# LouisBearing/BirdSoundClassif

Hardware: AMD Instinct MI355X
Metric: clips/sec (3 s @ 22.05 kHz) detect fwd (higher is better)
Workload: dtype f32; 1 GPU; BASELINE.json configs[1]: 1xMI355X inference, batch=64 synthetic 3 s clips (PCM16 @22.05 kHz resident in HBM) through the HIP STFT front end + detector forward + device post-processing, detections returned to the host; batch_per_gpu=64, distinct_clips=64, lanes=2

## Files before the change

### birdsoundclassif_amd/_lib.py

```python
import ctypes as C
import os
import subprocess

_HERE = os.path.dirname(os.path.abspath(__file__))
LIB_PATH = os.environ.get('NBM_LIB') or os.path.join(_HERE, 'libnbm_hip.so')
CSRC = os.path.join(_HERE, 'csrc')

_lib = None


class GemmDesc(C.Structure):
    _fields_ = [('x', C.c_void_p), ('w', C.c_void_p), ('y', C.c_void_p),
                ('scale', C.c_void_p), ('shift', C.c_void_p), ('residual', C.c_void_p),
                ('x_gs', C.c_int64), ('w_gs', C.c_int64), ('y_gs', C.c_int64), ('res_gs', C.c_int64),
                ('groups', C.c_int),
                ('B', C.c_int), ('H', C.c_int), ('W', C.c_int), ('Cin', C.c_int),
                ('N', C.c_int),
                ('kh', C.c_int), ('kw', C.c_int), ('stride', C.c_int), ('pad', C.c_int),
                ('Ho', C.c_int), ('Wo', C.c_int),
                ('x_ld', C.c_int), ('w_ld', C.c_int), ('y_ld', C.c_int), ('res_ld', C.c_int),
                ('alpha', C.c_float), ('act', C.c_int), ('shift_per_row', C.c_int),
                ('up', C.c_void_p), ('up_H', C.c_int), ('up_W', C.c_int),
                ('rows', C.c_void_p), ('rows_blocks', C.c_void_p),
                ('rows_mode', C.c_int), ('rows_count', C.c_int), ('rows_TH', C.c_int), ('rows_TW', C.c_int),
# ... 114 lines not shown
    'nbm_leaky_relu_bwd': [_P, _P, _P, _F, _L, _P],
    'nbm_layernorm_bwd': [_P, _P, _P, _L, _I, _F, _P, _P, _P, _P],
    'nbm_mha_small_bwd': [_P, _P, _P, _P, _I, _I, _I, _I, _P, _P, _P, _I, _I, _I, _P, _I, _I, _I, _I, _L, _L, _P, _F, _P],
    'nbm_layernorm_bwd_det': [_P, _P, _P, _L, _I, _F, _P, _P, _P, _P, _L, _P],
    'nbm_dropout': [_P, _P, _P, _L, _U32, _F, _U64, _U32, _U32, _P],
    'nbm_mha_small_drop': [_P, _P, _P, _I, _I, _I, _P, _I, _I, _I, _I, _I, _L, _L, _P, _F, _U32, _F, _U64, _U32, _U32, _P],
    'nbm_mha_small_drop_bwd': [_P, _P, _P, _P, _I, _I, _I, _I, _P, _P, _P, _I, _I, _I, _P, _I, _I, _I, _I, _L, _L, _P, _F,
                               _U32, _F, _U64, _U32, _U32, _P],
    'nbm_zero_roi_windows': [_P, _I, _I, _I, _P, _P, _I, _I, _I, _P],
    'nbm_zero_pattern': [_P, _I, _I, _I, _I, _I, _P],
    'nbm_zero_tiles': [_P, _I, _I, _I, _I, _P, _I, _P, _P],
    'nbm_tiles_gather': [_P, _I, _I, _I, _I, _P, _I, _P, _P, _P],
    'nbm_tiles_scatter_add': [_P, _I, _I, _I, _I, _P, _I, _P, _P, _P],
    'nbm_proposal_iou': [_P, _P, _P, _I, _I, _I, _P, _P, _P],
    'nbm_anchor_targets': [_P, _I, _P, _P, _I, _I, _F, _F, _P, _P, _P, _P],
    'nbm_maxpool3x3s2_bwd': [_P, _P, _P, _I, _I, _I, _I, _I, _I, _P, _P, _P],
    'nbm_upsample_bilinear_bwd': [_P, _I, _I, _I, _I, _P, _I, _I, _I, _P],
    'nbm_tiles_upsample_bilinear_bwd_add': [_P, _I, _I, _I, _I, _P, _I, _P, _P, _I, _I, _P],
    'nbm_png_unfilter_gray8': [_P, _L, _I, _I, _I, _P, _L, _P, _P],
    'nbm_png_inflate': [_P, _L, _P, _I, _P, _L, _L, _P, _P],
    'nbm_image_half_std_u8': [_P, _L, _I, _L, _P, _P],
    'nbm_randn_fill': [_U64, _L, _P, _P],
    'nbm_augment_batch': [_P, _P, _P, _I, _I, _I, _P, _P, _P, _P, _P, _P, _P],
    'nbm_u8_to_unit': [_P, _L, _P, _P],
    'nbm_wino_input': [_P, _I, _I, _I, _I, _P, _I, _P],
    'nbm_wino_output': [_P, _P, _P, _P, _I, _I, _I, _I, _I, _P, _I, _P, _P],
    'nbm_wino_outgrad': [_P, _I, _I, _I, _I, _P, _P, _I, _P],
    'nbm_wino_weight': [_P, _P, _I, _I, _I, _I, _P, _P],
    'nbm_wino_weight_grad': [_P, _P, _I, _I, _I, _P, _P],
    'nbm_wino23_rows': [_P, _I, _I, _I, _I, _P, _P],
    'nbm_wino23_conv_fused': [_P, _P, _P, _P, _P, _I, _I, _I, _I, _I, _I, _P, _I, _P],
    'nbm_wino23_rows_tiles': [_P, _I, _I, _I, _I, _P, _I, _P, _P, _P, _I, _P],
    'nbm_wino23_conv_fused_tiles': [_P, _P, _P, _P, _P, _I, _I, _I, _I, _I, _I, _P, _P, _I, _P, _P, _P],
    'nbm_roi_tiles': [_P, _P, _I, _I, _I, _I, _P, _P, _P, _I, _P, _P, _P],
    'nbm_wino23_input_tiles': [_P, _I, _I, _I, _I, _P, _I, _P, _P, _P],
    'nbm_wino23_outgrad_tiles': [_P, _I, _I, _I, _I, _P, _I, _P, _P, _P, _I, _P],
    'nbm_cell_outgrad': [_P, _I, _I, _I, _I, _I, _P, _P, _P],
    'nbm_cell_weight': [_P, _I, _I, _P, _I, _P, _I, _P],
    'nbm_cell_weight_fold': [_P, _P, _I, _I, _I, _I, _F, _P, _I, _P, _I, _P],
    'nbm_cell_weight_grad': [_P, _I, _I, _I, _P, _P],
    'nbm_cell_input': [_P, _I, _I, _I, _I, _I, _P, _I, _I, _P],
    'nbm_cell_input_up': [_P, _P, _I, _I, _I, _I, _I, _I, _I, _P, _I, _I, _P],
    'nbm_cell_patches': [_P, _I, _I, _I, _I, _I, _P, _I, _I, _P],
    'nbm_cell_patches_up': [_P, _P, _I, _I, _I, _I, _I, _I, _I, _P, _I, _I, _P],
    'nbm_cell_patches_up_cols': [_P, _P, _I, _I, _I, _I, _I, _I, _I, _P, _P],
    'nbm_cell_dgrad_output': [_P, _I, _I, _I, _I, _I, _P, _I, _I, _I, _P, _P],
    'nbm_cell_output': [_P, _P, _I, _I, _I, _I, _I, _P, _P],
    'nbm_weighted_sum': [_P, _P, _P, _P, _P, _L, _P],
    'nbm_weighted_sum_bwd': [_P, _P, _P, _P, _P, _P, _P, _P, _P, _L, _P],
    'nbm_softmax_rows_bwd': [_P, _P, _P, _L, _I, _F, _P],
    'nbm_pair_softmax_bwd': [_P, _P, _P, _L, _P],
    'nbm_dwconv3x3_bwd': [_P, _P, _P, _I, _I, _I, _I, _I, _I, _P, _P, _P, _I, _I, _P],
    'nbm_dwconv3x3_bwd_acc': [_P, _P, _I, _I, _I, _I, _I, _I, _P, _I, _I, _P],
    'nbm_film_fwd': [_P, _P, _P, _L, _I, _P],
    'nbm_film_bwd': [_P, _P, _P, _P, _P, _L, _I, _P],
    'nbm_bn_train_fwd': [_P, _L, _I, _P, _P, _F, _F, _P, _P, _P, _P, _P, _P, _P],
    'nbm_bn_train_bwd': [_P, _P, _L, _I, _P, _P, _P, _P, _P, _P, _P, _P],
    'nbm_bn_act_plan': [_L, _I, C.POINTER(C.c_int), C.POINTER(C.c_int64)],
    'nbm_bn_act_train_fwd': [_P, _L, _I, _P, _P, _F, _F, _P, _P, _P, _I, _P, _L, _P, _P, _P, _P],
    'nbm_bn_act_train_bwd': [_P, _P, _P, _L, _I, _P, _P, _P, _I, _P, _L, _P, _P, _P, _P, _P],
    'nbm_roi_pool_bwd': [C.POINTER(C.c_void_p), C.POINTER(C.c_int), C.POINTER(C.c_int), _I, _I, _P, _P, _I, _I, _P, _P],
    'nbm_roi_pool_hw_bwd': [C.POINTER(C.c_void_p), C.POINTER(C.c_int), C.POINTER(C.c_int), _I, _I, _P, _P, _I, _I, _I, _I, _P, _P],
    'nbm_sqnorm_accum': [_P, _L, _P, _P],
    'nbm_adamw_step': [_P, _P, _P, _P, _L, _F, _F, _F, _F, _F, _I, _P, _F, _P],
}

# ... 41 lines not shown
```

### birdsoundclassif_amd/csrc/wino_fused.hip

```cpp
#include "nbm_common.h"
#include "igemm_device.h"
#include <type_traits>

namespace {

constexpr int BK = 32;
constexpr int PITCH = 36;
constexpr int LIST_BM = 128;

struct WinoFusedParams {
  const float* R; const float* U; float* y;
  const float* scale; const float* shift; const float* mask;
  long long r_gs;
  int u_gs;
  int T, N, C, nk;
  int H, W, TH, TW, THW, WP;
  nbm_fastdiv fd_thw, fd_tw;
  int m_tiles, n_tiles, relu;
  const int* tiles; const int* n_blocks;
  const unsigned* blk_info;
};

__global__ __launch_bounds__(256) void wino23_rows_kernel(const float* __restrict__ x, int B, int H, int W, int C4,
                                                          int TH, int WP, float* __restrict__ R) {
  const long long per_plane = (long long)B * TH * WP * C4;
  const f32x4* x4 = reinterpret_cast<const f32x4*>(x);
  f32x4* r4 = reinterpret_cast<f32x4*>(R);
  const f32x4 zero = {0.f, 0.f, 0.f, 0.f};
  for (long long idx = blockIdx.x * 256ll + threadIdx.x; idx < per_plane; idx += (long long)gridDim.x * 256) {
    const int c = (int)(idx % C4);
    long long t = idx / C4;
    const int xp = (int)(t % WP);
    t /= WP;
    const int ty = (int)(t % TH), b = (int)(t / TH);
    const int ix = xp - 1;
    f32x4 d[4];
#pragma unroll
    for (int a = 0; a < 4; ++a) {
      const int iy = 2 * ty - 1 + a;
      const bool ok = (unsigned)iy < (unsigned)H && (unsigned)ix < (unsigned)W;
      d[a] = ok ? x4[(((long long)b * H + iy) * W + ix) * C4 + c] : zero;
    }
    r4[idx] = d[0] - d[2];
    r4[idx + per_plane] = d[1] + d[2];
    r4[idx + 2 * per_plane] = d[2] - d[1];
    r4[idx + 3 * per_plane] = d[1] - d[3];
  }
}

__global__ __launch_bounds__(256) void wino23_rows_tiles_kernel(const float* __restrict__ x, int B, int H, int W, int C4,
                                                                int TH, int TW, int WP, const int* __restrict__ tiles,
                                                                int n_entries, const int* __restrict__ n_blocks,
                                                                const unsigned* __restrict__ blk_info, float* __restrict__ R,
// ... 11 lines not shown
    const int k = (int)(t & 3), e = (int)(t >> 2);
    const int id = tiles[e];
    if (id < 0) continue;
    const unsigned pm = blk_info ? blk_info[e >> 7] & 0xffffu : 0xffffu;
    if ((k == 0 && !(pm & 0x1111u)) || (k == 3 && !(pm & 0x8888u))) continue;
    const int THW = TH * TW;
    const int b = id / THW, rem = id - b * THW;
    const int ty = rem / TW, tx = rem - ty * TW;
    const int xp = 2 * tx + k, ix = xp - 1;
    f32x4 d[4];
#pragma unroll
    for (int a = 0; a < 4; ++a) {
      const int iy = 2 * ty - 1 + a;
      bool ok = (unsigned)iy < (unsigned)H && (unsigned)ix < (unsigned)W &&
                !(a == 0 && !(pm & 0x000fu)) && !(a == 3 && !(pm & 0xf000u));
      if (S > 0 && ok && (iy + 1) % S < 3 && (iy + 1) / S < OHp && (ix + 1) % S < 3 && (ix + 1) / S < OWp) ok = false;
      d[a] = ok ? x4[(((long long)b * H + iy) * W + ix) * C4 + c] : zero;
    }
    const long long o = (((long long)b * TH + ty) * WP + xp) * C4 + c;
    if (pm & 0x000fu) r4[o] = d[0] - d[2];
    r4[o + per_plane] = d[1] + d[2];
    r4[o + 2 * per_plane] = d[2] - d[1];
    if (pm & 0xf000u) r4[o + 3 * per_plane] = d[1] - d[3];
  }
}

template <int BM, int BN, int WM, int WN>
__global__ __launch_bounds__(256, BN == 128 ? 1 : 2) void wino23_fused_kernel(const WinoFusedParams p) {
  constexpr int MT = WM / 32, NT = WN / 32;
  constexpr int WAVES_N = BN / WN;
  constexpr int AR = BM / 32, BR = BN / 32;
  static_assert((BM / WM) * WAVES_N == 4, "4 waves per workgroup");

  __shared__ __attribute__((aligned(16))) float lds[2 * (BM + BN) * PITCH];
  if constexpr (BN != 128) nbm_stagger_priority();
  float* As = lds;
  float* Bs = lds + 2 * BM * PITCH;

  const int wg = xcd_tile(gridDim.x, blockIdx.x);
  int tile_m = wg / p.n_tiles, tile_n = wg - tile_m * p.n_tiles;
  if (p.n_blocks) {
    const int j = blockIdx.x >> 3;
    tile_n = j % p.n_tiles;
    tile_m = (j / p.n_tiles) * 8 + (blockIdx.x & 7);
    if (tile_m >= p.m_tiles) return;
  }
  const int bm0 = tile_m * BM, bn0 = tile_n * BN;

  if (p.tiles) {
    if (p.n_blocks && tile_m >= *p.n_blocks) return;
    if (p.tiles[bm0] < 0) return;
  }
  auto tile_of = [&](int t) { return p.tiles ? p.tiles[t] : t; };
  const unsigned info = (p.tiles && p.blk_info) ? p.blk_info[tile_m] : 0x000fffffu;
  const unsigned plane_mask = info & 0xffffu, store_mask = (info >> 16) & 0xfu;

  const int tid = threadIdx.x, lane = tid & 63, wave = tid >> 6;
  const int wm0 = (wave / WAVES_N) * WM, wn0 = (wave % WAVES_N) * WN;
  const int lrow = lane & 31, lh = lane >> 5;
  const int c4 = tid & 7, r0 = tid >> 3;

  unsigned a_rel[AR], b_rel[BR];
  long long blk_base;
  {
    const int t = bm0 < p.T ? tile_of(bm0) : 0;
    const int bi = (int)nbm_fdiv((unsigned)t, p.fd_thw), rem = t - bi * p.THW;
    const int ty = (int)nbm_fdiv((unsigned)rem, p.fd_tw), tx = rem - ty * p.TW;
    blk_base = (((long long)bi * p.TH + ty) * p.WP + 2 * tx) * p.C;
  }
#pragma unroll
  for (int i = 0; i < AR; ++i) {
    const int t = bm0 + r0 + 32 * i < p.T ? tile_of(bm0 + r0 + 32 * i) : -1;
    if (t >= 0) {
      const int bi = (int)nbm_fdiv((unsigned)t, p.fd_thw), rem = t - bi * p.THW;
      const int ty = (int)nbm_fdiv((unsigned)rem, p.fd_tw), tx = rem - ty * p.TW;
      const long long off = (((long long)bi * p.TH + ty) * p.WP + 2 * tx) * p.C - blk_base;
      a_rel[i] = (unsigned)((off + c4 * 4) * 4);
    } else {
      a_rel[i] = 0x80000000u;
    }
  }
#pragma unroll
  for (int i = 0; i < BR; ++i) {
    const int n = bn0 + r0 + 32 * i;
    b_rel[i] = n < p.N ? (unsigned)((n * p.C + c4 * 4) * 4) : 0x80000000u;
  }
  const float* a_plane0 = p.R + blk_base;
  const __amdgpu_buffer_rsrc_t rsrc_b = make_rsrc(p.U, 0x7ffffff0u);

  f32x4 ra[AR], ra2[AR], rb[BR];
  float a_sign = 1.f;
  unsigned ld_rem = plane_mask;
  int ld_xi = __builtin_ctz(ld_rem), ld_c0 = 0;

  auto load_tiles = [&]() {
    const int i = ld_xi >> 2, j = ld_xi & 3;
    const int k1 = j == 0 ? 0 : (j == 2 ? 2 : 1), k2 = j == 2 ? 1 : (j == 3 ? 3 : 2);
    const __amdgpu_buffer_rsrc_t rsrc_a = make_rsrc(a_plane0 + (long long)i * p.r_gs, 0x7ffffff0u);
    const unsigned a_soff1 = (unsigned)((k1 * p.C + ld_c0) * 4), a_soff2 = (unsigned)((k2 * p.C + ld_c0) * 4);
    const unsigned b_soff = (unsigned)((ld_xi * p.u_gs + ld_c0) * 4);
#pragma unroll
    for (int r = 0; r < AR; ++r) {
      ra[r] = __builtin_bit_cast(f32x4, __builtin_amdgcn_raw_buffer_load_b128(rsrc_a, a_rel[r], a_soff1, 0));
      ra2[r] = __builtin_bit_cast(f32x4, __builtin_amdgcn_raw_buffer_load_b128(rsrc_a, a_rel[r], a_soff2, 0));
    }
#pragma unroll
    for (int r = 0; r < BR; ++r)
      rb[r] = __builtin_bit_cast(f32x4, __builtin_amdgcn_raw_buffer_load_b128(rsrc_b, b_rel[r], b_soff, 0));
    ld_c0 += BK;
    if (ld_c0 == p.C) { ld_c0 = 0; ld_rem &= ld_rem - 1; ld_xi = ld_rem ? __builtin_ctz(ld_rem) : 0; }
  };
  unsigned st_rem = plane_mask;
  int st_xi = __builtin_ctz(st_rem), st_c0 = 0;
  auto store_lds = [&](int buf) {
    const float sgn = (st_xi & 3) == 1 ? 1.f : -1.f;
#pragma unroll
    for (int r = 0; r < AR; ++r) {
      f32x4 v;
#pragma unroll
      for (int e = 0; e < 4; ++e) v[e] = fmaf(sgn, ra2[r][e], ra[r][e]);
      *reinterpret_cast<f32x4*>(As + (buf * BM + r0 + 32 * r) * PITCH + c4 * 4) = v;
    }
#pragma unroll
    for (int r = 0; r < BR; ++r)
      *reinterpret_cast<f32x4*>(Bs + (buf * BN + r0 + 32 * r) * PITCH + c4 * 4) = rb[r];
    st_c0 += BK;
    if (st_c0 == p.C) { st_c0 = 0; st_rem &= st_rem - 1; st_xi = st_rem ? __builtin_ctz(st_rem) : 0; }
  };
  (void)a_sign;

  f32x16 acc[MT][NT];
  f32x16 Y[2][2][MT][NT];
#pragma unroll
  for (int i = 0; i < MT; ++i)
#pragma unroll
    for (int j = 0; j < NT; ++j)
#pragma unroll
      for (int e = 0; e < 16; ++e) {
        acc[i][j][e] = 0.f;
        Y[0][0][i][j][e] = 0.f; Y[0][1][i][j][e] = 0.f; Y[1][0][i][j][e] = 0.f; Y[1][1][i][j][e] = 0.f;
      }

  f32x4 fa[2][MT], fb[2][NT];
  auto read_frags = [&](const float* Ab, const float* Bb, int q, int s) {
#pragma unroll
    for (int i = 0; i < MT; ++i) fa[s][i] = *reinterpret_cast<const f32x4*>(Ab + i * 32 * PITCH + q * 4);
#pragma unroll
    for (int j = 0; j < NT; ++j) fb[s][j] = *reinterpret_cast<const f32x4*>(Bb + j * 32 * PITCH + q * 4);
  };
  auto mfma_group = [&](int s) {
#pragma unroll
    for (int e = 0; e < 4; ++e)
#pragma unroll
      for (int i = 0; i < MT; ++i)
#pragma unroll
        for (int j = 0; j < NT; ++j)
          acc[i][j] = __builtin_amdgcn_mfma_f32_32x32x2f32(fa[s][i][e], fb[s][j][e], acc[i][j], 0, 0, 0);
  };

  int cur = 0;
  auto k_step = [&](auto store_c, auto load_c) {
    constexpr bool STORE = decltype(store_c)::value, LOAD = decltype(load_c)::value;
    constexpr int NM = 4 * MT * NT;
    __syncthreads();
    const float* Ab = As + (cur * BM + wm0 + lrow) * PITCH + lh * 16;
    const float* Bb = Bs + (cur * BN + wn0 + lrow) * PITCH + lh * 16;
    read_frags(Ab, Bb, 0, 0);
    read_frags(Ab, Bb, 1, 1);
    mfma_group(0);
    if constexpr (STORE) store_lds(cur ^ 1);
    __builtin_amdgcn_sched_group_barrier(0x100, 2 * (MT + NT), 0);
    if constexpr (STORE) {
#pragma unroll
      for (int z = 0; z < AR + BR; ++z) {
        __builtin_amdgcn_sched_group_barrier(0x008, NM / (AR + BR) > 0 ? NM / (AR + BR) : 1, 0);
        __builtin_amdgcn_sched_group_barrier(0x200, 1, 0);
      }
    }
    __builtin_amdgcn_sched_barrier(0);
    read_frags(Ab, Bb, 2, 0);
    mfma_group(1);
    if constexpr (LOAD) load_tiles();
    __builtin_amdgcn_sched_group_barrier(0x100, MT + NT, 0);
    if constexpr (LOAD) {
#pragma unroll
      for (int z = 0; z < 2 * AR + BR; ++z) {
        __builtin_amdgcn_sched_group_barrier(0x008, 1, 0);
        __builtin_amdgcn_sched_group_barrier(0x002, 2, 0);
        __builtin_amdgcn_sched_group_barrier(0x020, 1, 0);
      }
    }
    __builtin_amdgcn_sched_barrier(0);
// ... 4 lines not shown
    __builtin_amdgcn_sched_barrier(0);
    mfma_group(1);
    cur ^= 1;
  };

  auto flush = [&](int xi) {
    const int i = xi >> 2, j = xi & 3;
    const float ai[2] = {i < 3 ? 1.f : 0.f, i == 0 ? 0.f : (i == 1 ? 1.f : -1.f)};
    const float aj[2] = {j < 3 ? 1.f : 0.f, j == 0 ? 0.f : (j == 1 ? 1.f : -1.f)};
#pragma unroll
    for (int pp = 0; pp < 2; ++pp)
#pragma unroll
      for (int qq = 0; qq < 2; ++qq) {
        const float c = ai[pp] * aj[qq];
        if (c != 0.f) {
#pragma unroll
          for (int a = 0; a < MT; ++a)
#pragma unroll
            for (int b = 0; b < NT; ++b)
#pragma unroll
              for (int e = 0; e < 16; ++e) Y[pp][qq][a][b][e] = fmaf(c, acc[a][b][e], Y[pp][qq][a][b][e]);
        }
      }
#pragma unroll
    for (int a = 0; a < MT; ++a)
#pragma unroll
      for (int b = 0; b < NT; ++b)
#pragma unroll
        for (int e = 0; e < 16; ++e) acc[a][b][e] = 0.f;
  };

  using TT = std::true_type;
  using FF = std::false_type;
  load_tiles();
  store_lds(0);
  load_tiles();
  for (unsigned rem = plane_mask; rem;) {
    const int xi = __builtin_ctz(rem);
    rem &= rem - 1;
    if (rem) {
      for (int kt = 0; kt < p.nk; ++kt) k_step(TT{}, TT{});
    } else {
      for (int kt = 0; kt + 2 < p.nk; ++kt) k_step(TT{}, TT{});
      k_step(TT{}, FF{});
      k_step(FF{}, FF{});
    }
    flush(xi);
  }
  __syncthreads();

  constexpr int CP = BN + 4;
  static_assert(BM * CP + 2 * BM <= 2 * (BM + BN) * PITCH, "epilogue tile + row table must fit the operand buffers");
  float* Cs = lds;
  long long* row_pix = reinterpret_cast<long long*>(lds + BM * CP);
  if (tid < BM) {
    const int t = bm0 + tid < p.T ? tile_of(bm0 + tid) : -1;
    long long v = -1;
    if (t >= 0) {
      const int bi = (int)nbm_fdiv((unsigned)t, p.fd_thw), rem = t - bi * p.THW;
      const int ty = (int)nbm_fdiv((unsigned)rem, p.fd_tw), tx = rem - ty * p.TW;
      const long long pix = (p.relu & 4) ? (long long)(bm0 + tid) * 4 : ((long long)bi * p.H + 2 * ty) * p.W + 2 * tx;
      v = (pix << 2) | (2 * ty + 1 < p.H ? 2 : 0) | (2 * tx + 1 < p.W ? 1 : 0);
    }
    row_pix[tid] = v;
  }
  constexpr int CH = BN / 4;
  constexpr int RPP = 256 / CH;
  const int cc = tid % CH, rr = tid / CH;
  const int n = bn0 + cc * 4;
  f32x4 sc = {1.f, 1.f, 1.f, 1.f}, sh = {0.f, 0.f, 0.f, 0.f};
  if (n < p.N) {
    if (p.scale) sc = *reinterpret_cast<const f32x4*>(p.scale + n);
    if (p.shift) sh = *reinterpret_cast<const f32x4*>(p.shift + n);
  }
#pragma unroll
  for (int pp = 0; pp < 2; ++pp)
#pragma unroll
    for (int qq = 0; qq < 2; ++qq) {
      if (!((store_mask >> (2 * pp + qq)) & 1u)) continue;
      __syncthreads();
#pragma unroll
      for (int a = 0; a < MT; ++a)
#pragma unroll
        for (int b = 0; b < NT; ++b)
#pragma unroll
          for (int e = 0; e < 16; ++e)
            Cs[(wm0 + a * 32 + (e & 3) + 8 * (e >> 2) + 4 * lh) * CP + wn0 + b * 32 + lrow] = Y[pp][qq][a][b][e];
      __syncthreads();
      if (n < p.N) {
        const int need = (pp ? 2 : 0) | (qq ? 1 : 0);
#pragma unroll 4
        for (int r = rr; r < BM; r += RPP) {
          const long long rp = row_pix[r];
          if (rp < 0) break;
          if ((rp & need) != need) continue;
          f32x4 v = *reinterpret_cast<const f32x4*>(Cs + r * CP + cc * 4);
          const long long idx = ((rp >> 2) + ((p.relu & 4) ? pp * 2 + qq : pp * p.W + qq)) * p.N + n;
#pragma unroll
          for (int e = 0; e < 4; ++e) v[e] = v[e] * sc[e] + sh[e];
          if (p.relu & 1) {
#pragma unroll
            for (int e = 0; e < 4; ++e) v[e] = fmaxf(v[e], 0.f);
          }
          if (p.relu & 2) {
            const f32x4 o = *reinterpret_cast<const f32x4*>(p.y + idx);
            v[0] += o[0]; v[1] += o[1]; v[2] += o[2]; v[3] += o[3];
          }
          if (p.mask) {
            const f32x4 mk = *reinterpret_cast<const f32x4*>(p.mask + idx);
#pragma unroll
            for (int e = 0; e < 4; ++e) if (!(mk[e] > 0.f)) v[e] = 0.f;
          }
          *reinterpret_cast<f32x4*>(p.y + idx) = v;
        }
      }
    }
}

}

extern "C" int nbm_wino23_rows(const float* x, int B, int H, int W, int C, float* R, void* stream) {
  if (!x || !R || B <= 0 || H <= 0 || W <= 0 || C <= 0 || (C & 3)) return NBM_EINVAL;
  if (!nbm_aligned16(x) || !nbm_aligned16(R)) return NBM_EALIGN;
  const int TH = (H + 1) >> 1, TW = (W + 1) >> 1, WP = 2 * TW + 2;
  const long long n = (long long)B * TH * WP * (C / 4);
  long long g = (n + 255) / 256;
  if (g > 65536) g = 65536;
  hipLaunchKernelGGL(wino23_rows_kernel, dim3((unsigned)g), dim3(256), 0, (hipStream_t)stream, x, B, H, W, C / 4, TH, WP, R);
  return nbm_launch_status();
}

extern "C" int nbm_wino23_rows_tiles(const float* x, int B, int H, int W, int C, const int* tiles, int n_entries,
                                     const int* n_blocks, const unsigned* blk_info, float* R, int skip_pattern_stride,
                                     void* stream) {
  if (!x || !R || !tiles || B <= 0 || H <= 0 || W <= 0 || C <= 0 || (C & 3) || n_entries < 0 || skip_pattern_stride < 0) return NBM_EINVAL;
  if (!nbm_aligned16(x) || !nbm_aligned16(R)) return NBM_EALIGN;
  if (n_entries == 0) return NBM_OK;
  const int TH = (H + 1) >> 1, TW = (W + 1) >> 1, WP = 2 * TW + 2;
  const long long n = (long long)n_entries * 4 * (C / 4);
  long long g = (n + 255) / 256;
  if (g > 16384) g = 16384;
  hipLaunchKernelGGL(wino23_rows_tiles_kernel, dim3((unsigned)g), dim3(256), 0, (hipStream_t)stream, x, B, H, W, C / 4, TH, TW,
                     WP, tiles, n_entries, n_blocks, blk_info, R, skip_pattern_stride);
  return nbm_launch_status();
}

static int wino23_conv_fused_launch(const float* R, const float* U, const float* scale, const float* shift,
                                    const float* mask, int relu, int B, int H, int W, int C, int N, float* y,
                                    const int* tiles, int n_entries, const int* n_blocks, const unsigned* blk_info,
                                    int variant, void* stream);

extern "C" int nbm_wino23_conv_fused(const float* R, const float* U, const float* scale, const float* shift,
                                     const float* mask, int relu, int B, int H, int W, int C, int N, float* y,
                                     int variant, void* stream) {
  return wino23_conv_fused_launch(R, U, scale, shift, mask, relu, B, H, W, C, N, y, nullptr, 0, nullptr, nullptr, variant, stream);
}

extern "C" int nbm_wino23_conv_fused_tiles(const float* R, const float* U, const float* scale, const float* shift,
                                           const float* mask, int relu, int B, int H, int W, int C, int N, float* y,
                                           const int* tiles, int n_entries, const int* n_blocks, const unsigned* blk_info,
                                           void* stream) {
  if (!tiles || n_entries < 0 || (n_entries % LIST_BM)) return NBM_EINVAL;
  if (n_entries == 0) return NBM_OK;
  return wino23_conv_fused_launch(R, U, scale, shift, mask, relu, B, H, W, C, N, y, tiles, n_entries, n_blocks, blk_info, 0,
                                  stream);
}

static int wino23_conv_fused_launch(const float* R, const float* U, const float* scale, const float* shift,
                                    const float* mask, int relu, int B, int H, int W, int C, int N, float* y,
                                    const int* tiles, int n_entries, const int* n_blocks, const unsigned* blk_info,
                                    int variant, void* stream) {
  if (!R || !U || !y || B <= 0 || H <= 0 || W <= 0 || C <= 0 || N <= 0) return NBM_EINVAL;
  if ((C % BK) || C / BK < 2 || (N & 3)) return NBM_EUNSUPPORTED;
  if (!nbm_aligned16(R) || !nbm_aligned16(U) || !nbm_aligned16(y) || (shift && !nbm_aligned16(shift)) ||
      (scale && !nbm_aligned16(scale)) || (mask && !nbm_aligned16(mask)))
    return NBM_EALIGN;
  WinoFusedParams p{};
  p.TH = (H + 1) >> 1; p.TW = (W + 1) >> 1; p.THW = p.TH * p.TW; p.WP = 2 * p.TW + 2;
  p.fd_thw = nbm_fastdiv_make((unsigned)p.THW); p.fd_tw = nbm_fastdiv_make((unsigned)p.TW);
  const long long T = (long long)B * p.THW;
  if (T > 0x7fffff00ll || (long long)N * C * 16 * 4 > 0x7fffffffll) return NBM_EUNSUPPORTED;
  if ((130ll * p.WP + 4) * C * 4 > 0x7fffffffll) return NBM_EUNSUPPORTED;
  if (tiles && (long long)(B < 8 ? B : 8) * p.TH * p.WP * C * 4 > 0x7fffffffll) return NBM_EUNSUPPORTED;
  p.R = R; p.U = U; p.y = y; p.scale = scale; p.shift = shift; p.mask = mask; p.relu = relu;
  p.T = (int)T; p.N = N; p.C = C; p.nk = C / BK; p.H = H; p.W = W;
  p.r_gs = (long long)B * p.TH * p.WP * C; p.u_gs = N * C;
  p.m_tiles = (int)((T + LIST_BM - 1) / LIST_BM);
  p.tiles = tiles; p.n_blocks = n_blocks; p.blk_info = blk_info;
  if (tiles) { p.T = n_entries; p.m_tiles = n_entries / LIST_BM; }
  hipStream_t st = (hipStream_t)stream;
  if (variant != 0 && variant != 64 && variant != 128) return NBM_EINVAL;
  const bool wide = variant == 128 || (variant == 0 && N % 128 == 0);
  p.n_tiles = wide ? (N + 127) / 128 : (N + 63) / 64;
  int bm = LIST_BM;
  if (wide && !tiles) {
    const char* fe = getenv("NBM_WINO_BM");
    const int force = fe ? atoi(fe) : 0;
    static const int cus = [] { int dev = 0, n = 0; (void)hipGetDevice(&dev); (void)hipDeviceGetAttribute(&n, hipDeviceAttributeMultiprocessorCount, dev);
                                return n > 0 ? n : 256; }();
    const long long nt = p.n_tiles;
    const long long r128 = ((T + 127) / 128 * nt + cus - 1) / cus, r96 = ((T + 95) / 96 * nt + cus - 1) / cus;
    if (force == 96 || (force == 0 && r96 * 96 * 108 < r128 * 128 * 100)) bm = 96;
    if (force == 128) bm = 128;
    p.m_tiles = (int)((T + bm - 1) / bm);
  }
  const dim3 grid((n_blocks ? (p.m_tiles + 7) / 8 * 8 : p.m_tiles) * p.n_tiles), block(256);
#define NBM_WF(BM_, BN_, WM_, WN_) hipLaunchKernelGGL((wino23_fused_kernel<BM_, BN_, WM_, WN_>), grid, block, 0, st, p)
  if (!wide) NBM_WF(128, 64, 64, 32);
  else if (bm == 96) NBM_WF(96, 128, 96, 32);
  else NBM_WF(128, 128, 64, 64);
#undef NBM_WF
  return nbm_launch_status();
}
```

### include/nbm_hip.h

```cpp
#ifndef NBM_HIP_H
#define NBM_HIP_H

#include <stdint.h>

#ifdef __cplusplus
extern "C" {
#endif

#define NBM_OK 0
#define NBM_EINVAL (-1)
#define NBM_EALIGN (-2)
#define NBM_EUNSUPPORTED (-3)

#define NBM_ACT_NONE 0
#define NBM_ACT_RELU 1
#define NBM_ACT_SILU 2
#define NBM_ACT_LEAKY 3

const char* nbm_version(void);

int nbm_graph_census(void* graph, long long counts[6]);

typedef struct nbm_gemm_desc {
  const float* x;
// ... 50 lines not shown
  long long workspace_bytes;
  int B, H, W;
  int groups, Cg;
  int kh, kw, stride, pad;
  int Ho, Wo;
  int g_ld, y_ld, x_ld, out_ld;
  int accumulate;
  int splits;
} nbm_gconv_bwd_desc;
int nbm_gconv3x3_dgrad(const nbm_gconv_bwd_desc* d, void* stream);
int nbm_gconv3x3_wgrad(const nbm_gconv_bwd_desc* d, void* stream);
int nbm_gconv3x3_wgrad_workspace(const nbm_gconv_bwd_desc* d, long long* bytes);

int nbm_wino_input(const float* x, int B, int H, int W, int C, float* V, int m, void* stream);
int nbm_wino_output(const float* M, const float* scale, const float* shift, const float* mask, int relu, int B, int H, int W,
                    int N, float* y, int m, const float* residual, void* stream);
int nbm_wino_outgrad(const float* g, int B, int H, int W, int N, float* dM, float* bias_grad, int m, void* stream);

int nbm_wino_weight(const float* g, const float* scale, int N, int C, int transposed, int m, float* U, void* stream);
int nbm_wino_weight_grad(const float* dU, const float* row_scale, int N, int C, int m, float* dW, void* stream);

int nbm_wino23_rows(const float* x, int B, int H, int W, int C, float* R, void* stream);
int nbm_wino23_conv_fused(const float* R, const float* U, const float* scale, const float* shift, const float* mask,
                          int relu, int B, int H, int W, int C, int N, float* y, int variant, void* stream);

int nbm_wino23_rows_tiles(const float* x, int B, int H, int W, int C, const int* tiles, int n_entries, const int* n_blocks,
                          const unsigned* blk_info, float* R,
                          int skip_pattern_stride ,
                          void* stream);
int nbm_wino23_conv_fused_tiles(const float* R, const float* U, const float* scale, const float* shift, const float* mask,
                                int relu ,
                                int B, int H, int W, int C, int N, float* y, const int* tiles, int n_entries,
                                const int* n_blocks, const unsigned* blk_info, void* stream);
int nbm_roi_tiles(const float* rois, const int* n_roi, int B, int roi_cap, int n_levels, int level, const int* fh,
                  const int* fw, const unsigned char* skip, int dilate, int* tiles, int* n_blocks, void* stream);
int nbm_wino23_input_tiles(const float* x, int B, int H, int W, int C, const int* tiles, int n_list, const unsigned* plane_mask,
                           float* V, void* stream);
int nbm_wino23_outgrad_tiles(const float* g, int B, int H, int W, int N, const int* tiles, int n_list, const unsigned* plane_mask,
                             float* dM, float* bias_grad, int skip_pattern_stride, void* stream);
int nbm_cell_outgrad(const float* g, int B, int H, int W, int N, int stride, float* Vg, float* bias_grad, void* stream);
int nbm_cell_weight(const float* w, int N, int C, float* U_nc, int ld, float* U_cn, int ldt, void* stream);
int nbm_cell_weight_fold(const float* w, const float* w_lat, int wl_ld, int N, int C, int Cin, float alpha, float* U_nc, int ld,
                         float* U_cn, int ldt, void* stream);
int nbm_cell_weight_grad(const float* dU, int N, int C, int ld, float* dW, void* stream);
int nbm_cell_input(const float* x, int B, int H, int W, int C, int stride, float* Vx, int ld ,
                   int c_off , void* stream);
int nbm_cell_input_up(const float* x1, const float* bias, int B, int H, int W, int C, int Hc, int Wc, int stride, float* Vx, int ld,
                      int c_off, void* stream);
int nbm_cell_patches(const float* x, int B, int H, int W, int C, int stride, float* Vx, int ld, int c_off, void* stream);
int nbm_cell_patches_up(const float* x1, const float* bias, int B, int H, int W, int C, int Hc, int Wc, int stride, float* Vx, int ld,
                        int c_off, void* stream);
int nbm_cell_patches_up_cols(const float* x1, const float* bias, int B, int H, int W, int C, int Hc, int Wc, int stride, float* Vx,
                             void* stream);

int nbm_copy_rect(float* strided, float* packed, int64_t n_outer, int64_t outer_pitch, int n_rows, int64_t row_pitch, int64_t width,
                  int to_strided, int zero_strided, void* stream);
int nbm_cell_dgrad_output(const float* M, int B, int H, int W, int C, int stride, float* gx, int parity_class,
                          int ld , int c_off ,
                          float* bias_grad , void* stream);
int nbm_cell_output(const float* M, const float* bias, int B, int H, int W, int N, int stride, float* y, void* stream);


int nbm_pcm16_to_wave(const int16_t* pcm, int64_t pcm_ld, int batch, int n, int upsample,
                      const int32_t* hq, int64_t first, int64_t count, float* out, int64_t out_ld, int lead,
                      int pad_mode, void* stream);

// ... 296 lines not shown
```

Baseline: 1103 clips/s.

## Make Winograd fused conv kernel persistent with next-tile prefetch during epilogue

Result: no change. 1102 clips/s (-0.1%).

```diff
diff --git a/birdsoundclassif_amd/_lib.py b/birdsoundclassif_amd/_lib.py
--- a/birdsoundclassif_amd/_lib.py
+++ b/birdsoundclassif_amd/_lib.py
@@ -170,6 +170,7 @@
     'nbm_wino23_conv_fused': [_P, _P, _P, _P, _P, _I, _I, _I, _I, _I, _I, _P, _I, _P],
     'nbm_wino23_rows_tiles': [_P, _I, _I, _I, _I, _P, _I, _P, _P, _P, _I, _P],
     'nbm_wino23_conv_fused_tiles': [_P, _P, _P, _P, _P, _I, _I, _I, _I, _I, _I, _P, _P, _I, _P, _P, _P],
+    'nbm_wino23_conv_fused_grid': [_P, _P, _P, _P, _P, _I, _I, _I, _I, _I, _I, _P, _P, _I, _P, _P, _I, _I, _P],
     'nbm_roi_tiles': [_P, _P, _I, _I, _I, _I, _P, _P, _P, _I, _P, _P, _P],
     'nbm_wino23_input_tiles': [_P, _I, _I, _I, _I, _P, _I, _P, _P, _P],
     'nbm_wino23_outgrad_tiles': [_P, _I, _I, _I, _I, _P, _I, _P, _P, _P, _I, _P],
diff --git a/birdsoundclassif_amd/csrc/wino_fused.hip b/birdsoundclassif_amd/csrc/wino_fused.hip
--- a/birdsoundclassif_amd/csrc/wino_fused.hip
+++ b/birdsoundclassif_amd/csrc/wino_fused.hip
@@ -3,6 +3,14 @@
 #include <type_traits>
 
 namespace {
+
+#ifdef NBM_WINO_CYCLES
+#define WINO_CLK(t) do { __builtin_amdgcn_sched_barrier(0); t = clock64(); __builtin_amdgcn_sched_barrier(0); } while (0)
+#define WINO_ONLY(...) __VA_ARGS__
+#else
+#define WINO_CLK(t) do { } while (0)
+#define WINO_ONLY(...)
+#endif
 
 constexpr int BK = 32;
 constexpr int PITCH = 36;
@@ -19,6 +27,9 @@
   int m_tiles, n_tiles, relu;
   const int* tiles; const int* n_blocks;
   const unsigned* blk_info;
+#ifdef NBM_WINO_CYCLES
+  long long* cyc;
+#endif
 };
 
 __global__ __launch_bounds__(256) void wino23_rows_kernel(const float* __restrict__ x, int B, int H, int W, int C4,
@@ -96,66 +107,95 @@
   constexpr int AR = BM / 32, BR = BN / 32;
   static_assert((BM / WM) * WAVES_N == 4, "4 waves per workgroup");
 
-  __shared__ __attribute__((aligned(16))) float lds[2 * (BM + BN) * PITCH];
+  constexpr int CP = BN + 4;
+  constexpr int NCS = BN == 128 ? 2 : 1;
+  constexpr bool AHEAD = BN == 128;
+  constexpr int OPER_FLOATS = 2 * (BM + BN) * PITCH, EPI_FLOATS = NCS * BM * CP + 2 * BM;
+  __shared__ __attribute__((aligned(16))) float lds[OPER_FLOATS > EPI_FLOATS ? OPER_FLOATS : EPI_FLOATS];
   if constexpr (BN != 128) nbm_stagger_priority();
   float* As = lds;
   float* Bs = lds + 2 * BM * PITCH;
-
-  const int wg = xcd_tile(gridDim.x, blockIdx.x);
-  int tile_m = wg / p.n_tiles, tile_n = wg - tile_m * p.n_tiles;
-  if (p.n_blocks) {
-    const int j = blockIdx.x >> 3;
-    tile_n = j % p.n_tiles;
-    tile_m = (j / p.n_tiles) * 8 + (blockIdx.x & 7);
-    if (tile_m >= p.m_tiles) return;
-  }
-  const int bm0 = tile_m * BM, bn0 = tile_n * BN;
-
-  if (p.tiles) {
-    if (p.n_blocks && tile_m >= *p.n_blocks) return;
-    if (p.tiles[bm0] < 0) return;
-  }
-  auto tile_of = [&](int t) { return p.tiles ? p.tiles[t] : t; };
-  const unsigned info = (p.tiles && p.blk_info) ? p.blk_info[tile_m] : 0x000fffffu;
-  const unsigned plane_mask = info & 0xffffu, store_mask = (info >> 16) & 0xfu;
 
   const int tid = threadIdx.x, lane = tid & 63, wave = tid >> 6;
   const int wm0 = (wave / WAVES_N) * WM, wn0 = (wave % WAVES_N) * WN;
   const int lrow = lane & 31, lh = lane >> 5;
   const int c4 = tid & 7, r0 = tid >> 3;
 
+  typedef const volatile __attribute__((address_space(4))) WinoFusedParams* KernArgs;
+  auto kernargs = [] { return (KernArgs)__builtin_amdgcn_kernarg_segment_ptr(); };
+  int tile_m = 0, tile_n = 0;
+  auto next_block = [&](int v) {
+    KernArgs q = kernargs();
+    const int m_tiles = q->m_tiles, n_tiles = q->n_tiles;
+    const int* tiles = q->tiles;
+    const int* n_blocks = q->n_blocks;
+    const int n_virt = (n_blocks ? (m_tiles + 7) / 8 * 8 : m_tiles) * n_tiles;
+    for (; v < n_virt; v += gridDim.x) {
+      if (n_blocks) {
+        const int j = v >> 3;
+        tile_n = j % n_tiles;
+        tile_m = (j / n_tiles) * 8 + (v & 7);
+      } else {
+        const int wg = xcd_tile(n_virt, v);
+        tile_m = wg / n_tiles;
+        tile_n = wg - tile_m * n_tiles;
+      }
+      if (tile_m >= m_tiles) continue;
+      if (tiles && ((n_blocks && tile_m >= *n_blocks) || tiles[tile_m * BM] < 0)) continue;
+      return v;
+    }
+    return -1;
+  };
+
   unsigned a_rel[AR], b_rel[BR];
-  long long blk_base;
-  {
-    const int t = bm0 < p.T ? tile_of(bm0) : 0;
-    const int bi = (int)nbm_fdiv((unsigned)t, p.fd_thw), rem = t - bi * p.THW;
-    const int ty = (int)nbm_fdiv((unsigned)rem, p.fd_tw), tx = rem - ty * p.TW;
-    blk_base = (((long long)bi * p.TH + ty) * p.WP + 2 * tx) * p.C;
-  }
-#pragma unroll
-  for (int i = 0; i < AR; ++i) {
-    const int t = bm0 + r0 + 32 * i < p.T ? tile_of(bm0 + r0 + 32 * i) : -1;
-    if (t >= 0) {
-      const int bi = (int)nbm_fdiv((unsigned)t, p.fd_thw), rem = t - bi * p.THW;
-      const int ty = (int)nbm_fdiv((unsigned)rem, p.fd_tw), tx = rem - ty * p.TW;
-      const long long off = (((long long)bi * p.TH + ty) * p.WP + 2 * tx) * p.C - blk_base;
-      a_rel[i] = (unsigned)((off + c4 * 4) * 4);
-    } else {
-      a_rel[i] = 0x80000000u;
-    }
-  }
-#pragma unroll
-  for (int i = 0; i < BR; ++i) {
-    const int n = bn0 + r0 + 32 * i;
-    b_rel[i] = n < p.N ? (unsigned)((n * p.C + c4 * 4) * 4) : 0x80000000u;
-  }
-  const float* a_plane0 = p.R + blk_base;
+  const float* a_plane0 = p.R;
   const __amdgpu_buffer_rsrc_t rsrc_b = make_rsrc(p.U, 0x7ffffff0u);
+  int bm0 = 0, bn0 = 0;
+  unsigned plane_mask = 0xffffu, store_mask = 0xfu;
+  unsigned ld_rem = 0, st_rem = 0;
+  int ld_xi = 0, ld_c0 = 0;
+  int st_xi = 0, st_c0 = 0;
+  auto setup_block = [&]() {
+    KernArgs q = kernargs();
+    const int T = q->T, N = q->N, C = q->C, TH = q->TH, TW = q->TW, THW = q->THW, WP = q->WP;
+    const nbm_fastdiv fd_thw = {q->fd_thw.mul, q->fd_thw.sh1, q->fd_thw.sh2}, fd_tw = {q->fd_tw.mul, q->fd_tw.sh1, q->fd_tw.sh2};
+    const int* tiles = q->tiles;
+    const unsigned* blk_info = q->blk_info;
+    auto tile_at = [&](int t) { return tiles ? tiles[t] : t; };
+    bm0 = tile_m * BM; bn0 = tile_n * BN;
+    const unsigned info = (tiles && blk_info) ? blk_info[tile_m] : 0x000fffffu;
+    plane_mask = info & 0xffffu; store_mask = (info >> 16) & 0xfu;
+    long long blk_base;
+    {
+      const int t = bm0 < T ? tile_at(bm0) : 0;
+      const int bi = (int)nbm_fdiv((unsigned)t, fd_thw), rem = t - bi * THW;
+      const int ty = (int)nbm_fdiv((unsigned)rem, fd_tw), tx = rem - ty * TW;
+      blk_base = (((long long)bi * TH + ty) * WP + 2 * tx) * C;
+    }
+#pragma unroll
+    for (int i = 0; i < AR; ++i) {
+      const int t = bm0 + r0 + 32 * i < T ? tile_at(bm0 + r0 + 32 * i) : -1;
+      if (t >= 0) {
+        const int bi = (int)nbm_fdiv((unsigned)t, fd_thw), rem = t - bi * THW;
+        const int ty = (int)nbm_fdiv((unsigned)rem, fd_tw), tx = rem - ty * TW;
+        const long long off = (((long long)bi * TH + ty) * WP + 2 * tx) * C - blk_base;
+        a_rel[i] = (unsigned)((off + c4 * 4) * 4);
+      } else {
+        a_rel[i] = 0x80000000u;
+      }
+    }
+#pragma unroll
+    for (int i = 0; i < BR; ++i) {
+      const int n = bn0 + r0 + 32 * i;
+      b_rel[i] = n < N ? (unsigned)((n * C + c4 * 4) * 4) : 0x80000000u;
+    }
+    a_plane0 = q->R + blk_base;
+    ld_rem = st_rem = plane_mask;
+    ld_xi = st_xi = __builtin_ctz(plane_mask);
+    ld_c0 = st_c0 = 0;
+  };
 
   f32x4 ra[AR], ra2[AR], rb[BR];
-  float a_sign = 1.f;
-  unsigned ld_rem = plane_mask;
-  int ld_xi = __builtin_ctz(ld_rem), ld_c0 = 0;
 
   auto load_tiles = [&]() {
     const int i = ld_xi >> 2, j = ld_xi & 3;
@@ -174,8 +214,6 @@
     ld_c0 += BK;
     if (ld_c0 == p.C) { ld_c0 = 0; ld_rem &= ld_rem - 1; ld_xi = ld_rem ? __builtin_ctz(ld_rem) : 0; }
   };
-  unsigned st_rem = plane_mask;
-  int st_xi = __builtin_ctz(st_rem), st_c0 = 0;
   auto store_lds = [&](int buf) {
     const float sgn = (st_xi & 3) == 1 ? 1.f : -1.f;
 #pragma unroll
@@ -191,7 +229,6 @@
     st_c0 += BK;
     if (st_c0 == p.C) { st_c0 = 0; st_rem &= st_rem - 1; st_xi = st_rem ? __builtin_ctz(st_rem) : 0; }
   };
-  (void)a_sign;
 
   f32x16 acc[MT][NT];
   f32x16 Y[2][2][MT][NT];
@@ -200,10 +237,7 @@
 #pragma unroll
     for (int j = 0; j < NT; ++j)
 #pragma unroll
-      for (int e = 0; e < 16; ++e) {
-        acc[i][j][e] = 0.f;
-        Y[0][0][i][j][e] = 0.f; Y[0][1][i][j][e] = 0.f; Y[1][0][i][j][e] = 0.f; Y[1][1][i][j][e] = 0.f;
-      }
+      for (int e = 0; e < 16; ++e) acc[i][j][e] = 0.f;
 
   f32x4 fa[2][MT], fb[2][NT];
   auto read_frags = [&](const float* Ab, const float* Bb, int q, int s) {
@@ -222,6 +256,7 @@
           acc[i][j] = __builtin_amdgcn_mfma_f32_32x32x2f32(fa[s][i][e], fb[s][j][e], acc[i][j], 0, 0, 0);
   };
 
+  WINO_ONLY(long long t_blk = 0, t_k0 = 0, t_k1 = 0, t_f1 = 0, c_flush = 0);
   int cur = 0;
   auto k_step = [&](auto store_c, auto load_c) {
     constexpr bool STORE = decltype(store_c)::value, LOAD = decltype(load_c)::value;
@@ -292,89 +327,141 @@
 
   using TT = std::true_type;
   using FF = std::false_type;
+  int v = next_block(blockIdx.x);
+  if (v < 0) return;
+  setup_block();
   load_tiles();
-  store_lds(0);
-  load_tiles();
-  for (unsigned rem = plane_mask; rem;) {
-    const int xi = __builtin_ctz(rem);
-    rem &= rem - 1;
-    if (rem) {
-      for (int kt = 0; kt < p.nk; ++kt) k_step(TT{}, TT{});
-    } else {
-      for (int kt = 0; kt + 2 < p.nk; ++kt) k_step(TT{}, TT{});
-      k_step(TT{}, FF{});
-      k_step(FF{}, FF{});
-    }
-    flush(xi);
+  WINO_CLK(t_blk);
+  for (;;) {
+    const int e_bm0 = bm0, e_bn0 = bn0;
+    const unsigned e_store = store_mask;
+#pragma unroll
+    for (int i = 0; i < MT; ++i)
+#pragma unroll
+      for (int j = 0; j < NT; ++j)
+#pragma unroll
+        for (int e = 0; e < 16; ++e) { Y[0][0][i][j][e] = 0.f; Y[0][1][i][j][e] = 0.f; Y[1][0][i][j][e] = 0.f; Y[1][1][i][j][e] = 0.f; }
+    cur = 0;
+    store_lds(0);
+    load_tiles();
+    WINO_CLK(t_k0);
+    for (unsigned rem = plane_mask; rem;) {
+      const int xi = __builtin_ctz(rem);
+      rem &= rem - 1;
+      if (rem) {
+        for (int kt = 0; kt < p.nk; ++kt) k_step(TT{}, TT{});
+      } else {
+        for (int kt = 0; kt + 2 < p.nk; ++kt) k_step(TT{}, TT{});
+        k_step(TT{}, FF{});
+        k_step(FF{}, FF{});
+      }
+      WINO_CLK(t_k1);
+      flush(xi);
+      WINO_CLK(t_f1);
+      WINO_ONLY(c_flush += t_f1 - t_k1);
+    }
+    __syncthreads();
+
+    WINO_ONLY(const int v_this = v);
+    v = next_block(v + gridDim.x);
+    if constexpr (AHEAD) {
+      if (v >= 0) {
+        setup_block();
+        load_tiles();
+      }
+    }
+
+    long long* row_pix = reinterpret_cast<long long*>(lds + NCS * BM * CP);
+    KernArgs q = kernargs();
+    const int eT = q->T, eN = q->N, eH = q->H, eW = q->W, erelu = q->relu;
+    const int* etiles = q->tiles;
+    float* ey = q->y;
+    const float* emask = q->mask;
+    if (tid < BM) {
+      const int THW = q->THW, TW = q->TW;
+      const nbm_fastdiv fd_thw = {q->fd_thw.mul, q->fd_thw.sh1, q->fd_thw.sh2}, fd_tw = {q->fd_tw.mul, q->fd_tw.sh1, q->fd_tw.sh2};
+      const int t = e_bm0 + tid < eT ? (etiles ? etiles[e_bm0 + tid] : e_bm0 + tid) : -1;
+      long long rp = -1;
+      if (t >= 0) {
+        const int bi = (int)nbm_fdiv((unsigned)t, fd_thw), rem = t - bi * THW;
+        const int ty = (int)nbm_fdiv((unsigned)rem, fd_tw), tx = rem - ty * TW;
+        const long long pix = (erelu & 4) ? (long long)(e_bm0 + tid) * 4 : ((long long)bi * eH + 2 * ty) * eW + 2 * tx;
+        rp = (pix << 2) | (2 * ty + 1 < eH ? 2 : 0) | (2 * tx + 1 < eW ? 1 : 0);
+      }
+      row_pix[tid] = rp;
+    }
+    constexpr int CH = BN / 4;
+    constexpr int RPP = 256 / CH;
+    const int cc = tid % CH, rr = tid / CH;
+    const int n = e_bn0 + cc * 4;
+    f32x4 sc = {1.f, 1.f, 1.f, 1.f}, sh = {0.f, 0.f, 0.f, 0.f};
+    if (n < eN) {
+      const float* scale = q->scale;
+      const float* shift = q->shift;
+      if (scale) sc = *reinterpret_cast<const f32x4*>(scale + n);
+      if (shift) sh = *reinterpret_cast<const f32x4*>(shift + n);
+    }
+    float* Cs = lds;
+#pragma unroll
+    for (int pp = 0; pp < 2; ++pp)
+#pragma unroll
+      for (int qq = 0; qq < 2; ++qq) {
+        if (!((e_store >> (2 * pp + qq)) & 1u)) continue;
+        if constexpr (NCS == 1) __syncthreads();
+#pragma unroll
+        for (int a = 0; a < MT; ++a)
+#pragma unroll
+          for (int b = 0; b < NT; ++b)
+#pragma unroll
+            for (int e = 0; e < 16; ++e)
+              Cs[(wm0 + a * 32 + (e & 3) + 8 * (e >> 2) + 4 * lh) * CP + wn0 + b * 32 + lrow] = Y[pp][qq][a][b][e];
+        __syncthreads();
+        if (n < eN) {
+          const int need = (pp ? 2 : 0) | (qq ? 1 : 0);
+#pragma unroll 4
+          for (int r = rr; r < BM; r += RPP) {
+            const long long rp = row_pix[r];
+            if (rp < 0) break;
+            if ((rp & need) != need) continue;
+            f32x4 o4 = *reinterpret_cast<const f32x4*>(Cs + r * CP + cc * 4);
+            const long long idx = ((rp >> 2) + ((erelu & 4) ? pp * 2 + qq : pp * eW + qq)) * eN + n;
+#pragma unroll
+            for (int e = 0; e < 4; ++e) o4[e] = o4[e] * sc[e] + sh[e];
+            if (erelu & 1) {
+#pragma unroll
+              for (int e = 0; e < 4; ++e) o4[e] = fmaxf(o4[e], 0.f);
+            }
+            if (erelu & 2) {
+              const f32x4 o = *reinterpret_cast<const f32x4*>(ey + idx);
+              o4[0] += o[0]; o4[1] += o[1]; o4[2] += o[2]; o4[3] += o[3];
+            }
+            if (emask) {
+              const f32x4 mk = *reinterpret_cast<const f32x4*>(emask + idx);
+#pragma unroll
+              for (int e = 0; e < 4; ++e) if (!(mk[e] > 0.f)) o4[e] = 0.f;
+            }
+            *reinterpret_cast<f32x4*>(ey + idx) = o4;
+          }
+        }
+        if constexpr (NCS == 2) Cs = Cs == lds ? lds + BM * CP : lds;
+      }
+#ifdef NBM_WINO_CYCLES
+    {
+      const long long t_end = clock64();
+      if (tid == 0 && p.cyc) {
+        long long* c = p.cyc + 8ll * v_this;
+        c[0] = t_k0 - t_blk; c[1] = t_k1 - t_k0; c[2] = t_f1 - t_k1; c[3] = t_end - t_f1; c[4] = c_flush; c[5] = t_end - t_blk;
+      }
+      t_blk = t_end; c_flush = 0;
+    }
+#endif
+    if (v < 0) break;
+    if constexpr (!AHEAD) {
+      setup_block();
+      load_tiles();
+    }
+    __syncthreads();
   }
-  __syncthreads();
-
-  constexpr int CP = BN + 4;
-  static_assert(BM * CP + 2 * BM <= 2 * (BM + BN) * PITCH, "epilogue tile + row table must fit the operand buffers");
-  float* Cs = lds;
-  long long* row_pix = reinterpret_cast<long long*>(lds + BM * CP);
-  if (tid < BM) {
-    const int t = bm0 + tid < p.T ? tile_of(bm0 + tid) : -1;
-    long long v = -1;
-    if (t >= 0) {
-      const int bi = (int)nbm_fdiv((unsigned)t, p.fd_thw), rem = t - bi * p.THW;
-      const int ty = (int)nbm_fdiv((unsigned)rem, p.fd_tw), tx = rem - ty * p.TW;
-      const long long pix = (p.relu & 4) ? (long long)(bm0 + tid) * 4 : ((long long)bi * p.H + 2 * ty) * p.W + 2 * tx;
-      v = (pix << 2) | (2 * ty + 1 < p.H ? 2 : 0) | (2 * tx + 1 < p.W ? 1 : 0);
-    }
-    row_pix[tid] = v;
-  }
-  constexpr int CH = BN / 4;
-  constexpr int RPP = 256 / CH;
-  const int cc = tid % CH, rr = tid / CH;
-  const int n = bn0 + cc * 4;
-  f32x4 sc = {1.f, 1.f, 1.f, 1.f}, sh = {0.f, 0.f, 0.f, 0.f};
-  if (n < p.N) {
-    if (p.scale) sc = *reinterpret_cast<const f32x4*>(p.scale + n);
-    if (p.shift) sh = *reinterpret_cast<const f32x4*>(p.shift + n);
-  }
-#pragma unroll
-  for (int pp = 0; pp < 2; ++pp)
-#pragma unroll
-    for (int qq = 0; qq < 2; ++qq) {
-      if (!((store_mask >> (2 * pp + qq)) & 1u)) continue;
-      __syncthreads();
-#pragma unroll
-      for (int a = 0; a < MT; ++a)
-#pragma unroll
-        for (int b = 0; b < NT; ++b)
-#pragma unroll
-          for (int e = 0; e < 16; ++e)
-            Cs[(wm0 + a * 32 + (e & 3) + 8 * (e >> 2) + 4 * lh) * CP + wn0 + b * 32 + lrow] = Y[pp][qq][a][b][e];
-      __syncthreads();
-      if (n < p.N) {
-        const int need = (pp ? 2 : 0) | (qq ? 1 : 0);
-#pragma unroll 4
-        for (int r = rr; r < BM; r += RPP) {
-          const long long rp = row_pix[r];
-          if (rp < 0) break;
-          if ((rp & need) != need) continue;
-          f32x4 v = *reinterpret_cast<const f32x4*>(Cs + r * CP + cc * 4);
-          const long long idx = ((rp >> 2) + ((p.relu & 4) ? pp * 2 + qq : pp * p.W + qq)) * p.N + n;
-#pragma unroll
-          for (int e = 0; e < 4; ++e) v[e] = v[e] * sc[e] + sh[e];
-          if (p.relu & 1) {
-#pragma unroll
-            for (int e = 0; e < 4; ++e) v[e] = fmaxf(v[e], 0.f);
-          }
-          if (p.relu & 2) {
-            const f32x4 o = *reinterpret_cast<const f32x4*>(p.y + idx);
-            v[0] += o[0]; v[1] += o[1]; v[2] += o[2]; v[3] += o[3];
-          }
-          if (p.mask) {
-            const f32x4 mk = *reinterpret_cast<const f32x4*>(p.mask + idx);
-#pragma unroll
-            for (int e = 0; e < 4; ++e) if (!(mk[e] > 0.f)) v[e] = 0.f;
-          }
-          *reinterpret_cast<f32x4*>(p.y + idx) = v;
-        }
-      }
-    }
 }
 
 }
@@ -405,31 +492,33 @@
   return nbm_launch_status();
 }
 
-static int wino23_conv_fused_launch(const float* R, const float* U, const float* scale, const float* shift,
-                                    const float* mask, int relu, int B, int H, int W, int C, int N, float* y,
-                                    const int* tiles, int n_entries, const int* n_blocks, const unsigned* blk_info,
-                                    int variant, void* stream);
-
 extern "C" int nbm_wino23_conv_fused(const float* R, const float* U, const float* scale, const float* shift,
                                      const float* mask, int relu, int B, int H, int W, int C, int N, float* y,
                                      int variant, void* stream) {
-  return wino23_conv_fused_launch(R, U, scale, shift, mask, relu, B, H, W, C, N, y, nullptr, 0, nullptr, nullptr, variant, stream);
+  return nbm_wino23_conv_fused_grid(R, U, scale, shift, mask, relu, B, H, W, C, N, y, nullptr, 0, nullptr, nullptr, variant, 0, stream);
 }
 
 extern "C" int nbm_wino23_conv_fused_tiles(const float* R, const float* U, const float* scale, const float* shift,
                                            const float* mask, int relu, int B, int H, int W, int C, int N, float* y,
                                            const int* tiles, int n_entries, const int* n_blocks, const unsigned* blk_info,
                                            void* stream) {
-  if (!tiles || n_entries < 0 || (n_entries % LIST_BM)) return NBM_EINVAL;
-  if (n_entries == 0) return NBM_OK;
-  return wino23_conv_fused_launch(R, U, scale, shift, mask, relu, B, H, W, C, N, y, tiles, n_entries, n_blocks, blk_info, 0,
-                                  stream);
-}
-
-static int wino23_conv_fused_launch(const float* R, const float* U, const float* scale, const float* shift,
-                                    const float* mask, int relu, int B, int H, int W, int C, int N, float* y,
-                                    const int* tiles, int n_entries, const int* n_blocks, const unsigned* blk_info,
-                                    int variant, void* stream) {
+  if (!tiles) return NBM_EINVAL;
+  return nbm_wino23_conv_fused_grid(R, U, scale, shift, mask, relu, B, H, W, C, N, y, tiles, n_entries, n_blocks, blk_info, 0, 0, stream);
+}
+
+#ifdef NBM_WINO_CYCLES
+static long long* g_wino_cyc = nullptr;
+extern "C" int nbm_wino23_cycles_buffer(long long* buf) { g_wino_cyc = buf; return NBM_OK; }
+#endif
+
+extern "C" int nbm_wino23_conv_fused_grid(const float* R, const float* U, const float* scale, const float* shift,
+                                          const float* mask, int relu, int B, int H, int W, int C, int N, float* y,
+                                          const int* tiles, int n_entries, const int* n_blocks, const unsigned* blk_info,
+                                          int variant, int max_workgroups, void* stream) {
+  if (tiles && (n_entries < 0 || (n_entries % LIST_BM))) return NBM_EINVAL;
+  if (!tiles && (n_entries || n_blocks || blk_info)) return NBM_EINVAL;
+  if (max_workgroups < 0) return NBM_EINVAL;
+  if (tiles && n_entries == 0) return NBM_OK;
   if (!R || !U || !y || B <= 0 || H <= 0 || W <= 0 || C <= 0 || N <= 0) return NBM_EINVAL;
   if ((C % BK) || C / BK < 2 || (N & 3)) return NBM_EUNSUPPORTED;
   if (!nbm_aligned16(R) || !nbm_aligned16(U) || !nbm_aligned16(y) || (shift && !nbm_aligned16(shift)) ||
@@ -453,18 +542,24 @@
   const bool wide = variant == 128 || (variant == 0 && N % 128 == 0);
   p.n_tiles = wide ? (N + 127) / 128 : (N + 63) / 64;
   int bm = LIST_BM;
+  static const int cus = [] { int dev = 0, n = 0; (void)hipGetDevice(&dev); (void)hipDeviceGetAttribute(&n, hipDeviceAttributeMultiprocessorCount, dev);
+                              return n > 0 ? n : 256; }();
   if (wide && !tiles) {
     const char* fe = getenv("NBM_WINO_BM");
     const int force = fe ? atoi(fe) : 0;
-    static const int cus = [] { int dev = 0, n = 0; (void)hipGetDevice(&dev); (void)hipDeviceGetAttribute(&n, hipDeviceAttributeMultiprocessorCount, dev);
-                                return n > 0 ? n : 256; }();
     const long long nt = p.n_tiles;
     const long long r128 = ((T + 127) / 128 * nt + cus - 1) / cus, r96 = ((T + 95) / 96 * nt + cus - 1) / cus;
     if (force == 96 || (force == 0 && r96 * 96 * 108 < r128 * 128 * 100)) bm = 96;
     if (force == 128) bm = 128;
     p.m_tiles = (int)((T + bm - 1) / bm);
   }
-  const dim3 grid((n_blocks ? (p.m_tiles + 7) / 8 * 8 : p.m_tiles) * p.n_tiles), block(256);
+  long long wgs = (long long)(n_blocks ? (p.m_tiles + 7) / 8 * 8 : p.m_tiles) * p.n_tiles;
+  if (wide && !tiles && wgs > cus) wgs = cus >= 8 ? cus / 8 * 8 : cus;
+  if (max_workgroups > 0 && wgs > max_workgroups) wgs = max_workgroups;
+#ifdef NBM_WINO_CYCLES
+  p.cyc = g_wino_cyc;
+#endif
+  const dim3 grid((unsigned)wgs), block(256);
 #define NBM_WF(BM_, BN_, WM_, WN_) hipLaunchKernelGGL((wino23_fused_kernel<BM_, BN_, WM_, WN_>), grid, block, 0, st, p)
   if (!wide) NBM_WF(128, 64, 64, 32);
   else if (bm == 96) NBM_WF(96, 128, 96, 32);
diff --git a/include/nbm_hip.h b/include/nbm_hip.h
--- a/include/nbm_hip.h
+++ b/include/nbm_hip.h
@@ -106,6 +106,9 @@
                                 int relu ,
                                 int B, int H, int W, int C, int N, float* y, const int* tiles, int n_entries,
                                 const int* n_blocks, const unsigned* blk_info, void* stream);
+int nbm_wino23_conv_fused_grid(const float* R, const float* U, const float* scale, const float* shift, const float* mask,
+                               int relu, int B, int H, int W, int C, int N, float* y, const int* tiles, int n_entries,
+                               const int* n_blocks, const unsigned* blk_info, int variant, int max_workgroups, void* stream);
 int nbm_roi_tiles(const float* rois, const int* n_roi, int B, int roi_cap, int n_levels, int level, const int* fh,
                   const int* fw, const unsigned char* skip, int dilate, int* tiles, int* n_blocks, void* stream);
 int nbm_wino23_input_tiles(const float* x, int B, int H, int W, int C, const int* tiles, int n_list, const unsigned* plane_mask,
```
